# slp-rl/slamkit

Hardware: NVIDIA H100
Metric: speech-tokens/sec (SLAM seq=1024) (higher is better)
Workload: dtype bf16

## Files before the change

### slamkit_b200/csrc/attention.cu

```cuda
#include "kernels.h"

namespace {

constexpr int HD = 64;

SK_DEVINL uint32_t tile_addr(uint32_t base, int r, int chunk) { return base + r * 128 + ((chunk ^ (r & 7)) << 4); }
SK_DEVINL uint32_t smem_base_1k(const void* p) { return (smem_u32(p) + 1023u) & ~1023u; }

SK_DEVINL void cp_async16(uint32_t saddr, const void* g, bool pred) {
  const int sz = pred ? 16 : 0;
  asm volatile("cp.async.cg.shared.global [%0], [%1], 16, %2;" ::"r"(saddr), "l"(g), "r"(sz) : "memory");
}
SK_DEVINL void cp_async_commit() { asm volatile("cp.async.commit_group;" ::: "memory"); }
template <int N>
SK_DEVINL void cp_async_wait() {
  asm volatile("cp.async.wait_group %0;" ::"n"(N) : "memory");
}

SK_DEVINL void wgmma_m64n64_rs(float (&d)[32], const uint32_t (&a)[4], uint64_t db) {
  asm volatile(
      "{\n\t.reg .pred p;\n\tsetp.eq.u32 p, 1, 1;\n\t"
      "wgmma.mma_async.sync.aligned.m64n64k16.f32.bf16.bf16 {%0,%1,%2,%3,%4,%5,%6,%7,%8,%9,%10,%11,%12,%13,%14,%15,"
      "%16,%17,%18,%19,%20,%21,%22,%23,%24,%25,%26,%27,%28,%29,%30,%31}, {%32,%33,%34,%35}, %36, p, 1, 1, 1;\n\t}\n"
      : "+f"(d[0]), "+f"(d[1]), "+f"(d[2]), "+f"(d[3]), "+f"(d[4]), "+f"(d[5]), "+f"(d[6]), "+f"(d[7]), "+f"(d[8]),
// ... 18 lines not shown
  float(&d)[32] = reinterpret_cast<float(&)[32]>(acc);
  wgmma_fence();
#pragma unroll
  for (int ks = 0; ks < 4; ++ks)
    wgmma_m64n64<0, 0>(d, gmma_desc_sw128(sA + ks * 32, 16, 1024), gmma_desc_sw128(sB + ks * 32, 16, 1024));
  wgmma_commit();
  wgmma_wait<0>();
}

SK_DEVINL void wg_p_b(float (&acc)[8][4], const uint32_t (&p)[4][4], uint32_t sB) {
  float(&d)[32] = reinterpret_cast<float(&)[32]>(acc);
  wgmma_fence();
#pragma unroll
  for (int kk = 0; kk < 4; ++kk) wgmma_m64n64_rs(d, p[kk], gmma_desc_sw128(sB + kk * 2048, 8192, 1024));
  wgmma_commit();
  wgmma_wait<0>();
}

SK_DEVINL void acc_to_a(const float (&s)[8][4], uint32_t (&p)[4][4]) {
#pragma unroll
  for (int kk = 0; kk < 4; ++kk) {
    p[kk][0] = pack_bf16(s[2 * kk][0], s[2 * kk][1]);
    p[kk][1] = pack_bf16(s[2 * kk][2], s[2 * kk][3]);
    p[kk][2] = pack_bf16(s[2 * kk + 1][0], s[2 * kk + 1][1]);
    p[kk][3] = pack_bf16(s[2 * kk + 1][2], s[2 * kk + 1][3]);
  }
}

SK_DEVINL void zero_acc(float (&a)[8][4]) {
#pragma unroll
  for (int i = 0; i < 8; ++i)
#pragma unroll
    for (int j = 0; j < 4; ++j) a[i][j] = 0.f;
}

template <bool CAUSAL>
__global__ void __launch_bounds__(256, 2)
attn_fwd_kernel(const bf16* __restrict__ q, const bf16* __restrict__ k, const bf16* __restrict__ v, bf16* __restrict__ o,
                float* __restrict__ lse, int T, int ld, int ldo, int H, int group, float scale,
                const int* __restrict__ seg_start) {
  extern __shared__ __align__(128) uint8_t smem_attn[];
  const uint32_t sQ = smem_base_1k(smem_attn);
  const uint32_t sK = sQ + 128 * 128;
  const uint32_t sV = sK + 2 * 64 * 128;
  const int b = blockIdx.z, h = blockIdx.y;
  const int qt = gridDim.x - 1 - blockIdx.x;
  const int q0 = qt * 128;
  const int warp = threadIdx.x >> 5, lane = threadIdx.x & 31;
  const bf16* qp = q + (size_t)b * T * ld + h * HD;
  const bf16* kp = k + (size_t)b * T * ld + (h / group) * HD;
  const bf16* vp = v + (size_t)b * T * ld + (h / group) * HD;
  const float sl2 = scale * 1.4426950408889634f;

  int n_kv = (T + 63) / 64;
  if (CAUSAL) {
    const int last = min(T - 1, q0 + 127);
    n_kv = last / 64 + 1;
  }
  load_tile<128, 256>(sQ, qp, ld, q0, T);
  load_tile<64, 256>(sK, kp, ld, 0, T);
  load_tile<64, 256>(sV, vp, ld, 0, T);
  cp_async_commit();

  const uint32_t sQw = sQ + (uint32_t)(warp >> 2) * 8192u;
  float oacc[8][4];
  zero_acc(oacc);
// ... 249 lines not shown
    const long m = rh / H;
    const uint4 a = ldg128_stream(o + m * ldo + h * HD + part * 8);
    const uint4 g = ldg128_stream(d_o + m * ldo + h * HD + part * 8);
    const uint32_t au[4] = {a.x, a.y, a.z, a.w}, gu[4] = {g.x, g.y, g.z, g.w};
#pragma unroll
    for (int kq = 0; kq < 4; ++kq) {
      const float2 x = unpack_bf16(au[kq]), y = unpack_bf16(gu[kq]);
      acc += x.x * y.x + x.y * y.y;
    }
  }
  acc += __shfl_xor_sync(0xffffffffu, acc, 1);
  acc += __shfl_xor_sync(0xffffffffu, acc, 2);
  acc += __shfl_xor_sync(0xffffffffu, acc, 4);
  if (ok && (i & 7) == 0) {
    const int h = (int)(rh % H);
    const long m = rh / H;
    const long bb = m / T, t = m % T;
    delta[(bb * H + h) * T + t] = acc;
  }
}

template <bool CAUSAL>
__global__ void __launch_bounds__(128, 3)
attn_bwd_dkdv_kernel(const bf16* __restrict__ q, const bf16* __restrict__ k, const bf16* __restrict__ v,
                     const bf16* __restrict__ d_o, const float* __restrict__ lse, const float* __restrict__ delta,
                     bf16* __restrict__ dk, bf16* __restrict__ dv, int T, int ld, int ldo, int ldg, int H, int group,
                     float scale, const int* __restrict__ seg_start) {
  extern __shared__ __align__(128) uint8_t smem_attn[];
  const uint32_t sKV = smem_base_1k(smem_attn);
  const uint32_t sQ = sKV + 2 * 8192;
  const uint32_t sdO = sQ + 2 * 8192;
  float* sStat = reinterpret_cast<float*>(smem_attn + (sKV - smem_u32(smem_attn)) + 6 * 8192);
  int* sSeg = reinterpret_cast<int*>(sStat + 2 * 2 * 64);
  const int b = blockIdx.z, g = blockIdx.y;
  const int kt = blockIdx.x;
  const int k0 = kt * 64;
  const int warp = threadIdx.x >> 5, lane = threadIdx.x & 31;
  const float sl2 = scale * 1.4426950408889634f;
  const bf16* kp = k + (size_t)b * T * ld + g * HD;
  const bf16* vp = v + (size_t)b * T * ld + g * HD;

  load_tile<64, 128>(sKV, kp, ld, k0, T);
  load_tile<64, 128>(sKV + 8192, vp, ld, k0, T);
  cp_async_commit();

  const int n_qt = (T + 63) / 64;
  const int qt_begin = CAUSAL ? kt : 0;
  const int per_head = n_qt - qt_begin;
  const int n_iter = per_head * group;

  auto issue = [&](int it, int st) {
    const int h = g * group + it / per_head;
    const int qt = qt_begin + it % per_head;
    const bf16* qp = q + (size_t)b * T * ld + h * HD;
    const bf16* dop = d_o + (size_t)b * T * ldo + h * HD;
    load_tile<64, 128>(sQ + st * 8192, qp, ld, qt * 64, T);
    load_tile<64, 128>(sdO + st * 8192, dop, ldo, qt * 64, T);
    if (threadIdx.x < 64) {
      const int row = qt * 64 + threadIdx.x;
      const size_t off = ((size_t)b * H + h) * T + (row < T ? row : 0);
      sStat[(st * 2 + 0) * 64 + threadIdx.x] = row < T ? lse[off] : 0.f;
      sStat[(st * 2 + 1) * 64 + threadIdx.x] = row < T ? delta[off] : 0.f;
      sSeg[st * 64 + threadIdx.x] = (seg_start && row < T) ? seg_start[(size_t)b * T + row] : 0;
    }
    cp_async_commit();
  };
  if (n_iter > 0) issue(0, 0);

  float dkacc[8][4], dvacc[8][4];
  zero_acc(dkacc);
  zero_acc(dvacc);
  const int key_a = k0 + warp * 16 + (lane >> 2);

  for (int it = 0; it < n_iter; ++it) {
    const int st = it & 1;
    if (it + 1 < n_iter) {
      issue(it + 1, st ^ 1);
      cp_async_wait<1>();
    } else {
      cp_async_wait<0>();
    }
    __syncthreads();
    const int qt = qt_begin + it % per_head;
    const int q0 = qt * 64;
    const float* s_lse = sStat + (st * 2 + 0) * 64;
    const float* s_del = sStat + (st * 2 + 1) * 64;

    float st_acc[8][4];
    zero_acc(st_acc);
    wg_a_bT(st_acc, sKV, sQ + st * 8192);
    const int* s_seg = sSeg + st * 64;
    const bool need_mask = (CAUSAL && (q0 < k0 + 64)) || (q0 + 64 > T) || (k0 + 64 > T) || seg_start;
#pragma unroll
    for (int nt = 0; nt < 8; ++nt) {
#pragma unroll
      for (int e = 0; e < 4; ++e) {
        const int qi = nt * 8 + (lane & 3) * 2 + (e & 1);
        const int key = key_a + ((e >> 1) << 3);
        float pv = exp2f(st_acc[nt][e] * sl2 - s_lse[qi] * 1.4426950408889634f);
        if (need_mask) {
          const int qrow = q0 + qi;
          if (qrow >= T || key >= T || (CAUSAL && key > qrow) || key < s_seg[qi]) pv = 0.f;
        }
        st_acc[nt][e] = pv;
      }
    }
    uint32_t pa[4][4];
    acc_to_a(st_acc, pa);
    wg_p_b(dvacc, pa, sdO + st * 8192);

    float dp[8][4];
    zero_acc(dp);
    wg_a_bT(dp, sKV + 8192, sdO + st * 8192);
#pragma unroll
    for (int nt = 0; nt < 8; ++nt) {
#pragma unroll
      for (int e = 0; e < 4; ++e) {
        const int qi = nt * 8 + (lane & 3) * 2 + (e & 1);
        dp[nt][e] = st_acc[nt][e] * (dp[nt][e] - s_del[qi]) * scale;
      }
    }
    acc_to_a(dp, pa);
    wg_p_b(dkacc, pa, sQ + st * 8192);
    __syncthreads();
  }
#pragma unroll
  for (int r = 0; r < 2; ++r) {
    const int key = key_a + 8 * r;
    if (key < T) {
      bf16* dkp = dk + ((size_t)b * T + key) * ldg + g * HD;
      bf16* dvp = dv + ((size_t)b * T + key) * ldg + g * HD;
#pragma unroll
      for (int nt = 0; nt < 8; ++nt) {
        *reinterpret_cast<uint32_t*>(dkp + nt * 8 + (lane & 3) * 2) = pack_bf16(dkacc[nt][2 * r], dkacc[nt][2 * r + 1]);
        *reinterpret_cast<uint32_t*>(dvp + nt * 8 + (lane & 3) * 2) = pack_bf16(dvacc[nt][2 * r], dvacc[nt][2 * r + 1]);
      }
    }
  }
}

template <bool CAUSAL>
__global__ void __launch_bounds__(128)
attn_bwd_dq_kernel(const bf16* __restrict__ q, const bf16* __restrict__ k, const bf16* __restrict__ v,
                   const bf16* __restrict__ d_o, const float* __restrict__ lse, const float* __restrict__ delta,
                   bf16* __restrict__ dq, int T, int ld, int ldo, int ldg, int H, int group, float scale,
                   const int* __restrict__ seg_start) {
  extern __shared__ __align__(128) uint8_t smem_attn[];
  const uint32_t sQdO = smem_base_1k(smem_attn);
  const uint32_t sK = sQdO + 2 * 8192;
  const uint32_t sV = sK + 2 * 8192;
  const int b = blockIdx.z, h = blockIdx.y;
  const int qt = gridDim.x - 1 - blockIdx.x;
  const int q0 = qt * 64;
  const int warp = threadIdx.x >> 5, lane = threadIdx.x & 31;
  const float sl2 = scale * 1.4426950408889634f;
  const bf16* qp = q + (size_t)b * T * ld + h * HD;
  const bf16* dop = d_o + (size_t)b * T * ldo + h * HD;
  const bf16* kp = k + (size_t)b * T * ld + (h / group) * HD;
  const bf16* vp = v + (size_t)b * T * ld + (h / group) * HD;

  int n_kv = (T + 63) / 64;
  if (CAUSAL) n_kv = min(T - 1, q0 + 63) / 64 + 1;
  load_tile<64, 128>(sQdO, qp, ld, q0, T);
  load_tile<64, 128>(sQdO + 8192, dop, ldo, q0, T);
  load_tile<64, 128>(sK, kp, ld, 0, T);
  load_tile<64, 128>(sV, vp, ld, 0, T);
  cp_async_commit();

  const int row_a = q0 + warp * 16 + (lane >> 2);
  float lse_r[2], del_r[2];
  int seg_r[2];
#pragma unroll
  for (int r = 0; r < 2; ++r) {
    const int row = row_a + 8 * r;
    const size_t off = ((size_t)b * H + h) * T + (row < T ? row : 0);
    lse_r[r] = row < T ? lse[off] * 1.4426950408889634f : 0.f;
    del_r[r] = row < T ? delta[off] : 0.f;
    seg_r[r] = (seg_start && row < T) ? seg_start[(size_t)b * T + row] : 0;
  }
  float dqacc[8][4];
  zero_acc(dqacc);

  for (int j = 0; j < n_kv; ++j) {
    const int st = j & 1;
    if (j + 1 < n_kv) {
      load_tile<64, 128>(sK + (st ^ 1) * 8192, kp, ld, (j + 1) * 64, T);
      load_tile<64, 128>(sV + (st ^ 1) * 8192, vp, ld, (j + 1) * 64, T);
      cp_async_commit();
      cp_async_wait<1>();
    } else {
      cp_async_wait<0>();
    }
    __syncthreads();
    const int k0 = j * 64;
    float s[8][4];
    zero_acc(s);
    wg_a_bT(s, sQdO, sK + st * 8192);
    const bool need_mask = (CAUSAL && (k0 + 63 > q0 + warp * 16)) || (k0 + 64 > T) || (q0 + 64 > T) || seg_start;
#pragma unroll
    for (int nt = 0; nt < 8; ++nt) {
#pragma unroll
      for (int e = 0; e < 4; ++e) {
        float pv = exp2f(s[nt][e] * sl2 - lse_r[e >> 1]);
        if (need_mask) {
          const int key = k0 + nt * 8 + (lane & 3) * 2 + (e & 1);
          const int row = row_a + ((e >> 1) << 3);
          if (row >= T || key >= T || (CAUSAL && key > row) || key < seg_r[e >> 1]) pv = 0.f;
        }
        s[nt][e] = pv;
      }
    }
    float dp[8][4];
    zero_acc(dp);
    wg_a_bT(dp, sQdO + 8192, sV + st * 8192);
#pragma unroll
    for (int nt = 0; nt < 8; ++nt) {
#pragma unroll
      for (int e = 0; e < 4; ++e) dp[nt][e] = s[nt][e] * (dp[nt][e] - del_r[e >> 1]) * scale;
    }
    uint32_t pa[4][4];
    acc_to_a(dp, pa);
    wg_p_b(dqacc, pa, sK + st * 8192);
    __syncthreads();
  }
#pragma unroll
  for (int r = 0; r < 2; ++r) {
    const int row = row_a + 8 * r;
    if (row < T) {
      bf16* dqp = dq + ((size_t)b * T + row) * ldg + h * HD;
#pragma unroll
      for (int nt = 0; nt < 8; ++nt)
        *reinterpret_cast<uint32_t*>(dqp + nt * 8 + (lane & 3) * 2) = pack_bf16(dqacc[nt][2 * r], dqacc[nt][2 * r + 1]);
    }
  }
}

constexpr int FWD_SMEM = 128 * 128 + 4 * 8192 + 1024;
constexpr int DKDV_SMEM = 6 * 8192 + 2 * 2 * 64 * 4 + 2 * 64 * 4 + 1024;
constexpr int DQ_SMEM = 6 * 8192 + 1024;
constexpr int FWD_SPLIT_SMEM = 2 * 128 * 128 + 8 * 8192 + 1024;

template <typename K>
int set_smem(K kernel, int bytes) {
  SK_CUDA_CHECK(cudaFuncSetAttribute(kernel, cudaFuncAttributeMaxDynamicSharedMemorySize, bytes));
  return 0;
}

// ... 10 lines not shown
    if (set_smem(attn_fwd_kernel<true>, FWD_SMEM)) return -2;
    if (set_smem(attn_fwd_kernel<false>, FWD_SMEM)) return -2;
    init = true;
  }
  dim3 grid((T + 127) / 128, H, B);
  sk_prof_begin(1, s);
  if (causal) attn_fwd_kernel<true><<<grid, 256, FWD_SMEM, s>>>(q, k, v, o, lse, T, ld, ldo, H, H / KVH, scale, seg_start);
  else attn_fwd_kernel<false><<<grid, 256, FWD_SMEM, s>>>(q, k, v, o, lse, T, ld, ldo, H, H / KVH, scale, nullptr);
  sk_prof_end(s);
  SK_LAUNCH_CHECK();
  return 0;
}

int sk_attn_bwd_launch(const bf16* q, const bf16* k, const bf16* v, const bf16* o, const bf16* d_o, const float* lse,
                       float* delta, bf16* dq, bf16* dk, bf16* dv, int B, int T, int H, int KVH, int ld, int ldo,
                       int ldg, int causal, float scale, cudaStream_t s, const int* seg_start) {
  SK_REQUIRE(seg_start == nullptr || causal, "attention: document segments need the causal kernels");
  SK_REQUIRE(B > 0 && T > 0 && H > 0 && KVH > 0, "attention: bad shape B=%d T=%d H=%d KVH=%d", B, T, H, KVH);
  SK_REQUIRE(H % KVH == 0, "attention: H must be a multiple of KVH");
  SK_REQUIRE(ld % 8 == 0 && ldo % 8 == 0 && ldg % 2 == 0, "attention: ld and ldo must be multiples of 8 and ldg even");
  static bool init = false;
  if (!init) {
    if (set_smem(attn_bwd_dkdv_kernel<true>, DKDV_SMEM)) return -2;
    if (set_smem(attn_bwd_dkdv_kernel<false>, DKDV_SMEM)) return -2;
    if (set_smem(attn_bwd_dq_kernel<true>, DQ_SMEM)) return -2;
    if (set_smem(attn_bwd_dq_kernel<false>, DQ_SMEM)) return -2;
    init = true;
  }
  const long total = (long)B * T * H * 8;
  sk_prof_begin(1, s);
  SK_CUDA_CHECK(sk_launch_pdl(attn_delta_kernel, dim3((int)((total + 255) / 256)), dim3(256), (size_t)(0), s, o, d_o, delta, B, T, H, ldo));
  SK_LAUNCH_CHECK();
  const int group = H / KVH;
  dim3 g1((T + 63) / 64, KVH, B), g2((T + 63) / 64, H, B);
  if (causal) {
    attn_bwd_dkdv_kernel<true><<<g1, 128, DKDV_SMEM, s>>>(q, k, v, d_o, lse, delta, dk, dv, T, ld, ldo, ldg, H, group, scale,
                                                          seg_start);
    SK_LAUNCH_CHECK();
    attn_bwd_dq_kernel<true><<<g2, 128, DQ_SMEM, s>>>(q, k, v, d_o, lse, delta, dq, T, ld, ldo, ldg, H, group, scale, seg_start);
  } else {
    attn_bwd_dkdv_kernel<false><<<g1, 128, DKDV_SMEM, s>>>(q, k, v, d_o, lse, delta, dk, dv, T, ld, ldo, ldg, H, group, scale,
                                                           nullptr);
    SK_LAUNCH_CHECK();
    attn_bwd_dq_kernel<false><<<g2, 128, DQ_SMEM, s>>>(q, k, v, d_o, lse, delta, dq, T, ld, ldo, ldg, H, group, scale, nullptr);
  }
  sk_prof_end(s);
  SK_LAUNCH_CHECK();
  return 0;
}

int sk_attn_fwd_split_launch(const bf16* q_hi, const bf16* q_lo, const bf16* k_hi, const bf16* k_lo, const bf16* v_hi,
                             const bf16* v_lo, bf16* o_hi, bf16* o_lo, int B, int T, int H, int ld, int ldo, float scale,
                             cudaStream_t s) {
  SK_REQUIRE(B > 0 && T > 0 && H > 0, "attention: bad shape B=%d T=%d H=%d", B, T, H);
  SK_REQUIRE(ld % 8 == 0 && ldo % 8 == 0, "attention: leading dims must be multiples of 8");
  static bool init = false;
  if (!init) {
    if (set_smem(attn_fwd_split_kernel, FWD_SPLIT_SMEM)) return -2;
    init = true;
  }
  dim3 grid((T + 127) / 128, H, B);
  sk_prof_begin(1, s);
  attn_fwd_split_kernel<<<grid, 256, FWD_SPLIT_SMEM, s>>>(q_hi, q_lo, k_hi, k_lo, v_hi, v_lo, o_hi, o_lo, T, ld, ldo, scale);
  sk_prof_end(s);
  SK_LAUNCH_CHECK();
  return 0;
}
// ... 36 lines not shown
```

### slamkit_b200/csrc/gemm_tcgen05.cu

```cuda
#include "common.cuh"
#include <cudaTypedefs.h>
#include <stdio.h>
#include <mutex>
#include <type_traits>
#include <string.h>
#include <stdlib.h>
#include "kernels.h"
#include "../../include/slamkit_b200.h"

namespace {

constexpr int BM = 128;
constexpr int BK = 64;
constexpr int MMA_K = 16;
constexpr int GEMM_THREADS = 288;


struct GemmParams {
  int M, N, K;
  int batch;
  int a_mode;
  int passes;
  void* C;
  void* C_lo;
  int ldc;
  const void* bias;
  int bias_f32;
  const bf16* residual;
  const bf16* residual_lo;
  int ldr;
  int tiles_m, tiles_n;
  int out_f32;
  int round_before_res;
  int act;
  int col_gin, col_gout;
  int splits;
  float* splitk_ws;
  int tma_store;
  int pdl;
  int sk_units;
  int sk_groups;
  int sk_G;
  int sk_colunits;
  int sk_carry;
  int units, n_groups;
  float* sk_ws;
  uint32_t* sk_flags;
  int epi;
  const bf16* aux;
  int ld_aux;
  const bf16* rope_cos;
  const bf16* rope_sin;
  const int* rope_pos;
  int rope_T, rope_cols, rope_maxpos, rope_rot;
};

template <int BN, int EW = 4>
struct GemmCfg {
  static constexpr int A_BYTES = BM * BK * 2;
  static constexpr int B_ATOMS = (BN + 63) / 64;
  static constexpr int B_BYTES = B_ATOMS * 64 * BK * 2;
  static constexpr int STAGE_BYTES = A_BYTES + B_BYTES;
  static constexpr int STAGES = (BN > 128) ? 4 : (BN > 64 ? 6 : 8);
  static constexpr int STAGING_BYTES = 4 * 2 * 4096;
  static constexpr int BAR_BYTES = 256;
  static constexpr int SMEM_BYTES = STAGES * STAGE_BYTES + STAGING_BYTES + BAR_BYTES + 1024;
  static_assert(BN % 64 == 0 || (BN == 224 && EW == 4), "a 32-column tail chunk only on the 224-wide tile");
  static_assert(STAGES * STAGE_BYTES >= BM * BN * 4, "the parked fp32 accumulator must fit in the stage ring");
  static_assert(SMEM_BYTES <= 227 * 1024, "sm_90 allows 227 KB of shared memory per block");
};

// ... 17 lines not shown
template <int BN>
SK_DEVINL void acc_ld_32x32(uint32_t base, uint32_t ta, uint32_t (&r)[32]) {
  const int row = (int)(ta >> 16) + (int)(threadIdx.x & 31);
  const int c0 = (int)(ta & 0xffffu) >> 2;
#pragma unroll
  for (int i = 0; i < 8; ++i)
    asm volatile("ld.shared.v4.b32 {%0, %1, %2, %3}, [%4];"
                 : "=r"(r[4 * i]), "=r"(r[4 * i + 1]), "=r"(r[4 * i + 2]), "=r"(r[4 * i + 3])
                 : "r"(acc_chunk_addr<BN>(base, row, c0 + i)) : "memory");
}

SK_DEVINL uint32_t staging_addr(uint32_t sbuf, int lane, int j, bool tail) {
  return tail ? sbuf + (uint32_t)lane * 64u + (uint32_t)((j ^ ((lane >> 1) & 3)) << 4)
              : sbuf + (uint32_t)lane * 128u + (uint32_t)((j ^ (lane & 7)) << 4);
}

SK_DEVINL float gelu_erf(float y) {
  const float a = fabsf(y);
  float t;
  asm("rcp.approx.ftz.f32 %0, %1;" : "=f"(t) : "f"(fmaf(0.3275911f * 0.70710678118654752440f, a, 1.0f)));
  float s = fmaf(0.5f * 1.061405429f, t, 0.5f * -1.453152027f);
  s = fmaf(s, t, 0.5f * 1.421413741f);
  s = fmaf(s, t, 0.5f * -0.284496736f);
  s = fmaf(s, t, 0.5f * 0.254829592f);
  const float e = ex2_approx((y * y) * -0.72134752044448170368f);
  return fmaf(-a, (s * t) * e, fmaxf(y, 0.0f));
}

SK_DEVINL float gelu_exact(float x) { return x * 0.5f * (1.0f + erff(x * 0.70710678118654752440f)); }
SK_DEVINL float gelu_exact_grad(float x) {
  const float cdf = 0.5f * (1.0f + erff(x * 0.70710678118654752440f));
  const float pdf = expf(-0.5f * x * x) * 0.39894228040143267794f;
  return cdf + x * pdf;
}

template <bool SK>
struct WorkIter {
  int num_kb, splits, kb_per_split, total_items, tiles_n;
  int G, colunits, carry, units, n_groups, sk_groups, grp, mem;
  long sk_total, sk_cur, sk_end;
  int next_unit, next_item;
  int tile, split, kb_begin, kb_end, role;
  long unit_end_it;
  SK_DEVINL WorkIter(const GemmParams& p, int num_kb_, int kb_per_split_, int total_items_) {
    num_kb = num_kb_;
    splits = p.splits;
    kb_per_split = kb_per_split_;
    total_items = total_items_;
    tiles_n = p.tiles_n;
    G = p.sk_G;
    colunits = p.sk_colunits;
    carry = p.sk_carry;
    units = p.units;
    n_groups = p.n_groups;
    sk_groups = p.sk_groups;
    tile = split = kb_begin = kb_end = role = 0;
    unit_end_it = 0;
    sk_total = sk_cur = sk_end = 0;
    next_item = (int)blockIdx.x;
    next_unit = 0;
    grp = mem = 0;
    if (SK && p.sk_units > 0) {
      grp = (int)blockIdx.x / G;
      mem = (int)blockIdx.x - grp * G;
      next_item = total_items;
      next_unit = grp < n_groups ? p.sk_units + grp : units;
// ... 172 lines not shown

  const int warp = threadIdx.x >> 5;
  const int lane = threadIdx.x & 31;
  const int tiles_per_batch = p.tiles_m * p.tiles_n;
  const int total_items = tiles_per_batch * p.batch * p.splits;
  const int num_kb_total = (p.K + BK - 1) / BK;
  const int kb_per_split = (num_kb_total + p.splits - 1) / p.splits;
  constexpr uint32_t STAGE_TX = Cfg::A_BYTES + (B_MN ? Cfg::B_ATOMS * 64 * BK * 2 : BN * BK * 2);

  if (threadIdx.x == 0) {
    tma_prefetch_desc(&tmA);
    tma_prefetch_desc(&tmB);
    for (int s = 0; s < Cfg::STAGES; ++s) {
      mbar_init(full_bar(s), 1);
      mbar_init(empty_bar(s), 8);
    }
    mbar_init(acc_free, 1);
    fence_mbar_init();
  }
  __syncthreads();
  griddep_wait();

  if (warp == 8) {
    if (lane == 0) {
      const bool split = p.passes == 3;
      const int n_stage = split ? Cfg::STAGES / 2 : Cfg::STAGES;
      const uint32_t stage_bytes = split ? 2u * Cfg::STAGE_BYTES : (uint32_t)Cfg::STAGE_BYTES;
      int stage = 0;
      uint32_t phase = 0;
      uint32_t acc_phase = 0;
      bool first = true;
      WorkIter<SK> w(p, num_kb_total, kb_per_split, total_items);
      while (w.next()) {
        if (!first) {
          mbar_wait_nocall(acc_free, acc_phase);
          acc_phase ^= 1u;
        }
        first = false;
        const int bidx = w.tile / tiles_per_batch;
        const int r = w.tile - bidx * tiles_per_batch;
        const int m0 = (r / p.tiles_n) * BM;
        const int n_blk = r % p.tiles_n;
        const int n0 = n_blk * BN;
        for (int kb = w.kb_begin; kb < w.kb_end; ++kb) {
          mbar_wait_nocall(empty_bar(stage), phase ^ 1u);
          const uint32_t fb = full_bar(stage);
          mbar_arrive_expect_tx(fb, split ? 2u * STAGE_TX : STAGE_TX);
          for (int part = 0; part < (split ? 2 : 1); ++part) {
            const CUtensorMap* mapA = part ? &tmA_lo : &tmA;
            const CUtensorMap* mapB = part ? &tmB_lo : &tmB;
            const uint32_t sA = smem_base + stage * stage_bytes + part * Cfg::STAGE_BYTES;
            const uint32_t sB = sA + Cfg::A_BYTES;
            if (!A_MN) {
              if (p.a_mode & 2) {
                if (p.a_mode & 1) tma_load_3d(sA, mapA, fb, n_blk * 64, m0 + kb, bidx);
                else tma_load_3d(sA, mapA, fb, kb * BK, m0, bidx);
              } else {
                tma_load_2d(sA, mapA, fb, kb * BK, m0);
              }
            } else {
#pragma unroll
              for (int j = 0; j < BM / 64; ++j) tma_load_2d(sA + j * (BK * 128), mapA, fb, m0 + 64 * j, kb * BK);
            }
            if (!B_MN) {
              tma_load_2d(sB, mapB, fb, kb * BK, n0);
            } else {
#pragma unroll
              for (int j = 0; j < Cfg::B_ATOMS; ++j) tma_load_2d(sB + j * (BK * 128), mapB, fb, n0 + 64 * j, kb * BK);
            }
          }
          if (++stage == n_stage) { stage = 0; phase ^= 1u; }
        }
      }
    }
  } else {
    const int wg = warp >> 2;
    const int q = warp & 3;
    const int chalf = warp >> 2;
    const bool epi_warp = warp < EW;
    auto acc_ld = [&](uint32_t ta, uint32_t (&r)[32]) { acc_ld_32x32<BN>(smem_base, ta, r); };
    const bool split = p.passes == 3;
    const int n_stage = split ? Cfg::STAGES / 2 : Cfg::STAGES;
    const uint32_t stage_bytes = split ? 2u * Cfg::STAGE_BYTES : (uint32_t)Cfg::STAGE_BYTES;
    int stage = 0;
    uint32_t phase = 0;
    uint32_t store_cnt = 0;
    auto release_acc = [&] {
      fence_proxy_async();
      named_bar_sync(1, 256);
      if (threadIdx.x == 0) mbar_arrive(acc_free);
    };
    WorkIter<SK> w(p, num_kb_total, kb_per_split, total_items);
    while (w.next()) {
      {
        float acc[BN / 2];
#pragma unroll
        for (int i = 0; i < BN / 2; ++i) acc[i] = 0.f;
        if (SK && w.role == 3) {
          const int src = (int)blockIdx.x - w.G;
          if (threadIdx.x == 0) {
            for (int qq = 0; qq < 4; ++qq) {
              const uint32_t* f = p.sk_flags + src * 4 + qq;
              const uint64_t t0 = globaltimer_ns();
              while (ld_acquire_u32(f) == 0u) {
                __nanosleep(64);
                if (globaltimer_ns() - t0 > 8000000000ull) __trap();
              }
            }
            for (int qq = 0; qq < 4; ++qq) p.sk_flags[src * 4 + qq] = 0u;
          }
          named_bar_sync(1, 256);
          const float* slot = p.sk_ws + (size_t)src * SK_SLOT_FLOATS;
          const int r0 = 64 * wg + 16 * (warp & 3) + (lane >> 2);
#pragma unroll
          for (int j = 0; j < BN / 8; ++j) {
            const int col = 8 * j + 2 * (lane & 3);
#pragma unroll
            for (int h = 0; h < 2; ++h) {
              const float2 v = __ldcg(reinterpret_cast<const float2*>(slot + sk_slot_off(col >> 5, (col & 31) >> 2, r0 + 8 * h) +
                                                                      (col & 3)));
              acc[4 * j + 2 * h] = v.x;
              acc[4 * j + 2 * h + 1] = v.y;
            }
          }
        }
        const int k_iters = max(0, w.kb_end - w.kb_begin);
        int prev = -1;
        for (int kb = 0; kb < k_iters; ++kb) {
          mbar_wait_nocall(full_bar(stage), phase);
          wgmma_fence();
          const uint32_t s_hi = smem_base + stage * stage_bytes;
          for (int g = 0; g < (split ? 3 : 1); ++g) {
            const uint32_t sA = s_hi + (g == 2 ? Cfg::STAGE_BYTES : 0) + (uint32_t)wg * 8192u;
            const uint32_t sB = s_hi + Cfg::A_BYTES + (g == 1 ? Cfg::STAGE_BYTES : 0);
#pragma unroll
            for (int k = 0; k < BK / MMA_K; ++k) {
              const uint64_t adesc = A_MN ? gmma_desc_sw128(sA + k * (MMA_K * 128), BK * 128, 1024)
                                          : gmma_desc_sw128(sA + k * (MMA_K * 2), 16, 1024);
              const uint64_t bdesc = B_MN ? gmma_desc_sw128(sB + k * (MMA_K * 128), BK * 128, 1024)
                                          : gmma_desc_sw128(sB + k * (MMA_K * 2), 16, 1024);
              wgmma_bf16<BN, A_MN ? 1 : 0, B_MN ? 1 : 0>(acc, adesc, bdesc);
            }
          }
          wgmma_commit();
          wgmma_wait<1>();
          if (prev >= 0 && lane == 0) mbar_arrive(empty_bar(prev));
          prev = stage;
          if (++stage == n_stage) { stage = 0; phase ^= 1u; }
        }
        wgmma_wait<0>();
        if (prev >= 0 && lane == 0) mbar_arrive(empty_bar(prev));
        named_bar_sync(1, 256);
        acc_park<BN>(smem_base, acc, wg, warp & 3, lane);
        named_bar_sync(1, 256);
      }
      if (!epi_warp) {
        release_acc();
        continue;
      }
      const int split_idx = w.split;
      const int bidx = w.tile / tiles_per_batch;
      const int rr = w.tile - bidx * tiles_per_batch;
      const int m0 = (rr / p.tiles_n) * BM;
      const int n0 = (rr % p.tiles_n) * BN;
      if (!SK && p.tma_store && p.epi == 2) {
        const int lpiece = lane & 7, lrsub = lane >> 3;
        const uint32_t sX = staging_base + (uint32_t)warp * (EW == 4 ? 8192u : 4096u);
        constexpr int NCH = BN / 64 / CS;
        const int c_lo = chalf * NCH;
        auto piece_off = [&](int bidx, int m0, int n0, int c2, size_t ld) -> size_t {
          const int acol = n0 + c2 * 64;
          const int gcol = (acol >> 7) * 256 + (acol & 127) + lpiece * 8;
          return (((size_t)bidx * p.M + m0 + q * 32 + lrsub) * ld + gcol) * sizeof(bf16);
        };
        const size_t row4_in = (size_t)4 * p.ld_aux * sizeof(bf16), row4_out = (size_t)4 * p.ldc * sizeof(bf16);
        uint4 gv[8], uv[8];
        auto gu_load_k = [&](int k, const uint8_t* base, int m0, int n0, int c2) {
          const int rin = m0 + q * 32 + 4 * k + lrsub;
          if (rin < p.M && n0 + c2 * 64 < p.N) {
            gv[k] = ldg128(base + k * row4_in);
            uv[k] = ldg128(base + k * row4_in + 256);
          } else {
            gv[k] = make_uint4(0u, 0u, 0u, 0u);
            uv[k] = make_uint4(0u, 0u, 0u, 0u);
          }
        };
        {
          const uint8_t* base = reinterpret_cast<const uint8_t*>(p.aux) + piece_off(bidx, m0, n0, c_lo, (size_t)p.ld_aux);
// ... 462 lines not shown
                if (p.out_f32) {
                  float* dst = reinterpret_cast<float*>(p.C) + row * p.ldc + ocol;
                  *reinterpret_cast<float4*>(dst) = make_float4(v[0], v[1], v[2], v[3]);
                  *reinterpret_cast<float4*>(dst + 4) = make_float4(v[4], v[5], v[6], v[7]);
                } else {
                  uint4 o;
                  o.x = pack_bf16(v[0], v[1]);
                  o.y = pack_bf16(v[2], v[3]);
                  o.z = pack_bf16(v[4], v[5]);
                  o.w = pack_bf16(v[6], v[7]);
                  stg128(reinterpret_cast<bf16*>(p.C) + row * p.ldc + ocol, o);
                  if (p.C_lo) {
                    const float2 h0 = unpack_bf16(o.x), h1 = unpack_bf16(o.y), h2 = unpack_bf16(o.z), h3 = unpack_bf16(o.w);
                    uint4 l;
                    l.x = pack_bf16(v[0] - h0.x, v[1] - h0.y);
                    l.y = pack_bf16(v[2] - h1.x, v[3] - h1.y);
                    l.z = pack_bf16(v[4] - h2.x, v[5] - h2.y);
                    l.w = pack_bf16(v[6] - h3.x, v[7] - h3.y);
                    stg128(reinterpret_cast<bf16*>(p.C_lo) + row * p.ldc + ocol, l);
                  }
                }
              }
            }
          }
        }
        if (SK && w.role == 2) {
          __syncwarp();
          if (lane == 0)
            for (int i = 0; i < n_contrib; ++i) p.sk_flags[(first_contrib + i * w.G) * 4 + q] = 0u;
        }
      }
      release_acc();
    }
    if (epi_warp && p.tma_store && lane == 0) tma_store_wait<0>();
  }
}

__global__ void splitk_reduce_kernel(const float* __restrict__ ws, bf16* __restrict__ C, int M, int N, int ldc, int splits,
                                     int accumulate, int round_before_res) {
  griddep_launch();
  griddep_wait();
  const long total = (long)M * N / 8;
  for (long i = blockIdx.x * (long)blockDim.x + threadIdx.x; i < total; i += (long)gridDim.x * blockDim.x) {
    const long e = i * 8;
    const int m = (int)(e / N), n = (int)(e % N);
    float acc[8] = {0, 0, 0, 0, 0, 0, 0, 0};
    for (int s = 0; s < splits; ++s) {
      const float* src = ws + ((size_t)s * M + m) * N + n;
      const float4 a = *reinterpret_cast<const float4*>(src), b = *reinterpret_cast<const float4*>(src + 4);
      acc[0] += a.x; acc[1] += a.y; acc[2] += a.z; acc[3] += a.w;
      acc[4] += b.x; acc[5] += b.y; acc[6] += b.z; acc[7] += b.w;
    }
    bf16* dst = C + (size_t)m * ldc + n;
    if (accumulate) {
      const uint4 o = *reinterpret_cast<const uint4*>(dst);
      const uint32_t ow[4] = {o.x, o.y, o.z, o.w};
#pragma unroll
      for (int k = 0; k < 4; ++k) {
        const float2 f = unpack_bf16(ow[k]);
        acc[2 * k] = (round_before_res ? bf16_round(acc[2 * k]) : acc[2 * k]) + f.x;
        acc[2 * k + 1] = (round_before_res ? bf16_round(acc[2 * k + 1]) : acc[2 * k + 1]) + f.y;
      }
    }
    stg128(dst, make_uint4(pack_bf16(acc[0], acc[1]), pack_bf16(acc[2], acc[3]), pack_bf16(acc[4], acc[5]),
                           pack_bf16(acc[6], acc[7])));
  }
}
// ... 234 lines not shown
    }
  }
  p.sk_G = 1;
  if (sk_ok && BN == 256 && p.splits == 1 && num_kb >= sk_min_kb && (p.tiles_n <= 8 || p.tiles_m <= 8)) {
    const int colunits = p.tiles_n <= 8 ? 0 : 1;
    const int G = colunits ? p.tiles_m : p.tiles_n;
    const int units = colunits ? p.tiles_n : p.tiles_m;
    const int n_groups = nsm / G;
    const int rem = units % n_groups;
    const long slots = ((long)(units + n_groups - 1) / n_groups) * n_groups;
    const bool multiwave = units > n_groups;
    if (n_groups >= 1 && rem != 0 && (slots - units) * 100 >= slots * sk_min_idle &&
        (!colunits || multiwave || sk_env >= 2)) {
      if (colunits && multiwave) {
        p.sk_units = rem + n_groups;
        p.sk_groups = n_groups;
        p.sk_carry = 1;
      } else {
        p.sk_units = rem;
        p.sk_groups = n_groups < rem * sk_ranges ? n_groups : rem * sk_ranges;
      }
      p.sk_G = G;
      p.sk_colunits = colunits;
      p.units = units;
      p.n_groups = n_groups;
      p.sk_ws = reinterpret_cast<float*>(g.splitk_ws);
      p.sk_flags = reinterpret_cast<uint32_t*>(reinterpret_cast<uint8_t*>(g.splitk_ws) + ws_data_bytes);
    }
  }
  const long work = tiles * p.splits;
  grid = p.sk_units > 0 ? p.n_groups * p.sk_G : (int)(work < nsm ? work : nsm);
  static const int ew_env = [] { const char* e = getenv("SK_GEMM_EW"); return e ? atoi(e) : 0; }();
  ew = (p.sk_units == 0 && BN == 256 && p.tma_store && (ew_env == 8 || (ew_env == 0 && (g.epi == 2 || g.epi == 3 || g.epi == 4 || g.epi == 5)))) ? 8 : 4;
  return 0;
}

}

int sk_gemm_plan_ex(const SkGemmEx& g, SkGemmPlan* out) {
  GemmParams p;
  int BN = 0, ew = 0, grid = 0;
  const int rc = plan_gemm(g, p, BN, ew, grid);
  if (rc) return rc;
  out->bn = BN;
  out->epi_warps = ew;
  out->splits = p.splits;
  out->sk_units = p.sk_units;
  out->sk_groups = p.sk_groups;
  out->sk_G = p.sk_G;
  out->sk_colunits = p.sk_colunits;
  out->tma_store = p.tma_store;
  out->grid = grid;
  return 0;
}

int sk_gemm_ex_launch(const SkGemmEx& g, cudaStream_t stream) {
  GemmParams p;
  int BN = 0, ew = 0, grid = 0;
  const int rc0 = plan_gemm(g, p, BN, ew, grid);
  if (rc0) return rc0;
  const bool use3d = g.a_rows > 0;
  CUtensorMap tm[6];
  const void* As[2] = {g.A, g.passes == 3 ? g.A_lo : g.A};
  const void* Bs[2] = {g.B, g.passes == 3 ? g.B_lo : g.B};
  for (int i = 0; i < 2; ++i) {
    int rc;
    CUtensorMap* ta = &tm[i == 0 ? 0 : 2];
    CUtensorMap* tb = &tm[i == 0 ? 1 : 3];
    if (use3d) {
      rc = sk_make_tmap_3d(ta, As[i], (uint64_t)g.a_inner, (uint64_t)g.a_rows, (uint64_t)g.batch, (uint64_t)g.a_row_stride,
                           (uint64_t)g.a_batch_stride, BM);
    } else if (!g.a_mn) {
      rc = sk_make_tmap_2d(ta, As[i], 2, (uint64_t)g.K, (uint64_t)g.M, (uint64_t)g.lda, BK, BM);
    } else {
      rc = sk_make_tmap_2d(ta, As[i], 2, (uint64_t)g.M, (uint64_t)g.K, (uint64_t)g.lda, 64, BK);
    }
    if (rc) return rc;
    if (!g.b_mn) rc = sk_make_tmap_2d(tb, Bs[i], 2, (uint64_t)g.K, (uint64_t)g.N, (uint64_t)g.ldb, BK, (uint32_t)BN);
    else         rc = sk_make_tmap_2d(tb, Bs[i], 2, (uint64_t)g.N, (uint64_t)g.K, (uint64_t)g.ldb, 64, BK);
    if (rc) return rc;
  }
  tm[4] = tm[0];
  if (p.tma_store) {
    const int rc2 = sk_make_tmap_2d(&tm[4], g.C, 2, (uint64_t)(g.epi == 2 ? 2 * g.N : g.N), (uint64_t)g.M, (uint64_t)g.ldc, 64, 32);
    if (rc2) return rc2;
  }
  tm[5] = tm[4];
  if (g.epi == 1) {
    const int rc3 = sk_make_tmap_2d(&tm[5], g.aux_out, 2, (uint64_t)g.N / 2, (uint64_t)g.M, (uint64_t)g.ld_aux_out, 64, 32);
    if (rc3) return rc3;
  } else if (g.epi == 4) {
    const int rc3 = sk_make_tmap_2d(&tm[5], g.aux_out, 2, (uint64_t)g.N, (uint64_t)g.M, (uint64_t)g.ld_aux_out, 64, 32);
    if (rc3) return rc3;
  } else if (p.tma_store && BN % 64 != 0) {
    const int rc3 = sk_make_tmap_2d(&tm[5], g.C, 2, (uint64_t)g.N, (uint64_t)g.M, (uint64_t)g.ldc, 32, 32);
    if (rc3) return rc3;
  }
  int rc;
  if (p.sk_units > 0) {
    rc = dispatch_major<256, true>(g.a_mn, g.b_mn, tm, p, grid, stream);
  } else if (ew == 8) {
    rc = dispatch_major<256, false, 8>(g.a_mn, g.b_mn, tm, p, grid, stream);
  } else {
    switch (BN) {
      case 256: rc = dispatch_major<256, false>(g.a_mn, g.b_mn, tm, p, grid, stream); break;
      case 224: rc = dispatch_major<224, false>(g.a_mn, g.b_mn, tm, p, grid, stream); break;
      case 192: rc = dispatch_major<192, false>(g.a_mn, g.b_mn, tm, p, grid, stream); break;
      case 128: rc = dispatch_major<128, false>(g.a_mn, g.b_mn, tm, p, grid, stream); break;
      default:  rc = dispatch_major<64, false>(g.a_mn, g.b_mn, tm, p, grid, stream); break;
    }
  }
  if (rc) return rc;
  if (p.splits > 1) {
    SK_REQUIRE(g.residual == nullptr || g.residual == g.C, "gemm: split-K supports only in-place accumulation");
    const long n8 = (long)g.M * g.N / 8;
    int blocks = (int)((n8 + 255) / 256);
    if (blocks > sk_num_sms() * 8) blocks = sk_num_sms() * 8;
    sk_prof_begin(0, stream);
    SK_CUDA_CHECK(sk_launch_pdl(splitk_reduce_kernel, dim3(blocks), dim3(256), (size_t)(0), stream, p.splitk_ws, reinterpret_cast<bf16*>(g.C), g.M, g.N, g.ldc, p.splits,
                                                     g.residual != nullptr, g.round_before_res));
    sk_prof_end(stream);
    SK_LAUNCH_CHECK();
  }
  return 0;
}

SkGemmEx sk_gemm_desc(int M, int N, int K, const void* A, int lda, int a_mn, const void* B, int ldb, int b_mn, void* C,
                      int ldc, int out_f32, const void* bias, const void* residual, int ldr, int round_before_res, int act,
// ... 85 lines not shown
```

Measured before the change: 153,700.

## Overlap independent wgmma groups in attention backward and reorder dK/dV grid

In both backward kernels the S=QK^T and dP=dO·V^T matmuls are now issued back to back as separate async wgmma groups. The softmax/mask math on the first runs while the second is still in flight, and in dK/dV the dV update is also issued asynchronously before dS is computed. The dK/dV grid is flattened to one dimension with key tile as the slowest index, which changes the scheduling order across heads and batches. The dQ kernel gets a min-blocks launch bound of 4, which raises register pressure because two accumulators are now live at once.

```diff
diff --git a/slamkit_b200/csrc/attention.cu b/slamkit_b200/csrc/attention.cu
--- a/slamkit_b200/csrc/attention.cu
+++ b/slamkit_b200/csrc/attention.cu
@@ -74,6 +74,21 @@
   for (int i = 0; i < 8; ++i)
 #pragma unroll
     for (int j = 0; j < 4; ++j) a[i][j] = 0.f;
+}
+
+SK_DEVINL void wg_a_bT_async(float (&acc)[8][4], uint32_t sA, uint32_t sB) {
+  float(&d)[32] = reinterpret_cast<float(&)[32]>(acc);
+#pragma unroll
+  for (int ks = 0; ks < 4; ++ks)
+    wgmma_m64n64<0, 0>(d, gmma_desc_sw128(sA + ks * 32, 16, 1024), gmma_desc_sw128(sB + ks * 32, 16, 1024));
+  wgmma_commit();
+}
+
+SK_DEVINL void acc_fence(float (&a)[8][4]) {
+#pragma unroll
+  for (int i = 0; i < 8; ++i)
+#pragma unroll
+    for (int j = 0; j < 4; ++j) asm volatile("" : "+f"(a[i][j])::"memory");
 }
 
 template <bool CAUSAL>
@@ -389,8 +404,11 @@
   const uint32_t sdO = sQ + 2 * 8192;
   float* sStat = reinterpret_cast<float*>(smem_attn + (sKV - smem_u32(smem_attn)) + 6 * 8192);
   int* sSeg = reinterpret_cast<int*>(sStat + 2 * 2 * 64);
-  const int b = blockIdx.z, g = blockIdx.y;
-  const int kt = blockIdx.x;
+  const int n_qt = (T + 63) / 64;
+  const int kvh = H / group;
+  const int per_kt = gridDim.x / n_qt;
+  const int kt = blockIdx.x / per_kt;
+  const int g = blockIdx.x % per_kt % kvh, b = blockIdx.x % per_kt / kvh;
   const int k0 = kt * 64;
   const int warp = threadIdx.x >> 5, lane = threadIdx.x & 31;
   const float sl2 = scale * 1.4426950408889634f;
@@ -401,7 +419,6 @@
   load_tile<64, 128>(sKV + 8192, vp, ld, k0, T);
   cp_async_commit();
 
-  const int n_qt = (T + 63) / 64;
   const int qt_begin = CAUSAL ? kt : 0;
   const int per_head = n_qt - qt_begin;
   const int n_iter = per_head * group;
@@ -444,8 +461,16 @@
     const float* s_del = sStat + (st * 2 + 1) * 64;
 
     float st_acc[8][4];
+    float dp[8][4];
     zero_acc(st_acc);
-    wg_a_bT(st_acc, sKV, sQ + st * 8192);
+    zero_acc(dp);
+    acc_fence(st_acc);
+    acc_fence(dp);
+    wgmma_fence();
+    wg_a_bT_async(st_acc, sKV, sQ + st * 8192);
+    wg_a_bT_async(dp, sKV + 8192, sdO + st * 8192);
+    wgmma_wait<1>();
+    acc_fence(st_acc);
     const int* s_seg = sSeg + st * 64;
     const bool need_mask = (CAUSAL && (q0 < k0 + 64)) || (q0 + 64 > T) || (k0 + 64 > T) || seg_start;
 #pragma unroll
@@ -464,11 +489,16 @@
     }
     uint32_t pa[4][4];
     acc_to_a(st_acc, pa);
-    wg_p_b(dvacc, pa, sdO + st * 8192);
-
-    float dp[8][4];
-    zero_acc(dp);
-    wg_a_bT(dp, sKV + 8192, sdO + st * 8192);
+    wgmma_fence();
+    {
+      float(&d)[32] = reinterpret_cast<float(&)[32]>(dvacc);
+#pragma unroll
+      for (int kk = 0; kk < 4; ++kk)
+        wgmma_m64n64_rs(d, pa[kk], gmma_desc_sw128(sdO + st * 8192 + kk * 2048, 8192, 1024));
+      wgmma_commit();
+    }
+    wgmma_wait<1>();
+    acc_fence(dp);
 #pragma unroll
     for (int nt = 0; nt < 8; ++nt) {
 #pragma unroll
@@ -477,6 +507,7 @@
         dp[nt][e] = st_acc[nt][e] * (dp[nt][e] - s_del[qi]) * scale;
       }
     }
+    wgmma_wait<0>();
     acc_to_a(dp, pa);
     wg_p_b(dkacc, pa, sQ + st * 8192);
     __syncthreads();
@@ -497,7 +528,7 @@
 }
 
 template <bool CAUSAL>
-__global__ void __launch_bounds__(128)
+__global__ void __launch_bounds__(128, 4)
 attn_bwd_dq_kernel(const bf16* __restrict__ q, const bf16* __restrict__ k, const bf16* __restrict__ v,
                    const bf16* __restrict__ d_o, const float* __restrict__ lse, const float* __restrict__ delta,
                    bf16* __restrict__ dq, int T, int ld, int ldo, int ldg, int H, int group, float scale,
@@ -550,9 +581,16 @@
     }
     __syncthreads();
     const int k0 = j * 64;
-    float s[8][4];
+    float s[8][4], dp[8][4];
     zero_acc(s);
-    wg_a_bT(s, sQdO, sK + st * 8192);
+    zero_acc(dp);
+    acc_fence(s);
+    acc_fence(dp);
+    wgmma_fence();
+    wg_a_bT_async(s, sQdO, sK + st * 8192);
+    wg_a_bT_async(dp, sQdO + 8192, sV + st * 8192);
+    wgmma_wait<1>();
+    acc_fence(s);
     const bool need_mask = (CAUSAL && (k0 + 63 > q0 + warp * 16)) || (k0 + 64 > T) || (q0 + 64 > T) || seg_start;
 #pragma unroll
     for (int nt = 0; nt < 8; ++nt) {
@@ -567,9 +605,8 @@
         s[nt][e] = pv;
       }
     }
-    float dp[8][4];
-    zero_acc(dp);
-    wg_a_bT(dp, sQdO + 8192, sV + st * 8192);
+    wgmma_wait<0>();
+    acc_fence(dp);
 #pragma unroll
     for (int nt = 0; nt < 8; ++nt) {
 #pragma unroll
@@ -646,7 +683,9 @@
   SK_CUDA_CHECK(sk_launch_pdl(attn_delta_kernel, dim3((int)((total + 255) / 256)), dim3(256), (size_t)(0), s, o, d_o, delta, B, T, H, ldo));
   SK_LAUNCH_CHECK();
   const int group = H / KVH;
-  dim3 g1((T + 63) / 64, KVH, B), g2((T + 63) / 64, H, B);
+  const long n_dkdv = (long)((T + 63) / 64) * KVH * B;
+  SK_REQUIRE(n_dkdv < (1l << 31), "attention: %ld dK/dV tiles exceed one grid dimension", n_dkdv);
+  dim3 g1((unsigned)n_dkdv), g2((T + 63) / 64, H, B);
   if (causal) {
     attn_bwd_dkdv_kernel<true><<<g1, 128, DKDV_SMEM, s>>>(q, k, v, d_o, lse, delta, dk, dv, T, ld, ldo, ldg, H, group, scale,
                                                           seg_start);
```

Result: no change. 155,200 (median of 6 runs) (+0.9%).

## Store GEMM epilogue directly from registers via stmatrix and TMA, skipping accumulator park

Applied to the files above, without the earlier changes.

For plain and SwiGLU-gated epilogues with no bias, activation or residual, the math warpgroups now pack accumulators to bf16 themselves. They write them into per-warp staging buffers with stmatrix and issue 16-row TMA stores. This removes the shared-memory accumulator park, the handoff to separate epilogue warps, and the producer's wait on acc_free. In exchange, consumer warps now spend time on the epilogue, so the next tile's mainloop no longer overlaps with the previous tile's stores. The staging-buffer layout and swizzle must also match the new 16-row TMA box.

```diff
diff --git a/slamkit_b200/csrc/gemm_tcgen05.cu b/slamkit_b200/csrc/gemm_tcgen05.cu
--- a/slamkit_b200/csrc/gemm_tcgen05.cu
+++ b/slamkit_b200/csrc/gemm_tcgen05.cu
@@ -37,6 +37,7 @@
   int splits;
   float* splitk_ws;
   int tma_store;
+  int reg_epi;
   int pdl;
   int sk_units;
   int sk_groups;
@@ -120,6 +121,11 @@
   const float cdf = 0.5f * (1.0f + erff(x * 0.70710678118654752440f));
   const float pdf = expf(-0.5f * x * x) * 0.39894228040143267794f;
   return cdf + x * pdf;
+}
+
+SK_DEVINL void stmatrix_x4(uint32_t addr, uint32_t a, uint32_t b, uint32_t c, uint32_t d) {
+  asm volatile("stmatrix.sync.aligned.m8n8.x4.shared.b16 [%0], {%1, %2, %3, %4};" ::"r"(addr), "r"(a), "r"(b), "r"(c),
+               "r"(d) : "memory");
 }
 
 template <bool SK>
@@ -358,7 +364,7 @@
       bool first = true;
       WorkIter<SK> w(p, num_kb_total, kb_per_split, total_items);
       while (w.next()) {
-        if (!first) {
+        if (!first && !p.reg_epi) {
           mbar_wait_nocall(acc_free, acc_phase);
           acc_phase ^= 1u;
         }
@@ -419,10 +425,104 @@
     WorkIter<SK> w(p, num_kb_total, kb_per_split, total_items);
     while (w.next()) {
       {
-        float acc[BN / 2];
-#pragma unroll
-        for (int i = 0; i < BN / 2; ++i) acc[i] = 0.f;
+        auto reg_epilogue = [&](const float (&acc)[BN / 2]) {
+          const int rr = w.tile;
+          const int m0 = (rr / p.tiles_n) * BM, n0 = (rr % p.tiles_n) * BN;
+          const int row0 = m0 + 16 * warp;
+          const uint32_t stg = staging_base + (uint32_t)warp * 4096u;
+          auto emit = [&](const uint32_t (&pk)[16], const CUtensorMap* map, int col, bool tail) {
+            const uint32_t sbuf = stg + (store_cnt & 1u) * 2048u;
+            if (lane == 0) tma_store_wait_read<1>();
+            __syncwarp();
+            const int srow = (lane & 7) + (lane & 8);
+#pragma unroll
+            for (int jj = 0; jj < (tail ? 4 : 8); jj += 2) {
+              const int ch = jj + (lane >> 4);
+              const uint32_t addr = tail ? sbuf + (uint32_t)srow * 64u + (uint32_t)((ch ^ ((srow >> 1) & 3)) << 4)
+                                         : sbuf + (uint32_t)srow * 128u + (uint32_t)((ch ^ (srow & 7)) << 4);
+              stmatrix_x4(addr, pk[2 * jj], pk[2 * jj + 1], pk[2 * jj + 2], pk[2 * jj + 3]);
+            }
+            fence_proxy_async();
+            __syncwarp();
+            if (lane == 0) {
+              tma_store_2d(map, sbuf, col, row0);
+              tma_store_commit();
+            }
+            ++store_cnt;
+          };
+          auto pair_bf16 = [&](int j, int h) { return pack_bf16(acc[4 * j + 2 * h], acc[4 * j + 2 * h + 1]); };
+          if (p.epi == 1) {
+            if constexpr (BN == 256) {
+#pragma unroll
+              for (int i = 0; i < 2; ++i) {
+                uint32_t pk[16];
+#pragma unroll
+                for (int t = 0; t < 16; ++t) pk[t] = pair_bf16(8 * i + (t >> 1), t & 1);
+                emit(pk, &tmC, n0 + 64 * i, false);
+#pragma unroll
+                for (int t = 0; t < 16; ++t) pk[t] = pair_bf16(16 + 8 * i + (t >> 1), t & 1);
+                emit(pk, &tmC, n0 + 128 + 64 * i, false);
+#pragma unroll
+                for (int t = 0; t < 16; ++t) {
+                  const float2 gf = unpack_bf16(pair_bf16(8 * i + (t >> 1), t & 1));
+                  const float2 uf = unpack_bf16(pair_bf16(16 + 8 * i + (t >> 1), t & 1));
+                  const float2 sb = unpack_bf16(pack_bf16(silu_f(gf.x), silu_f(gf.y)));
+                  pk[t] = pack_bf16(sb.x * uf.x, sb.y * uf.y);
+                }
+                emit(pk, &tmAux, (n0 >> 1) + 64 * i, false);
+              }
+            }
+          } else {
+#pragma unroll
+            for (int c2 = 0; c2 < (BN + 63) / 64; ++c2) {
+              const bool tail = BN % 64 != 0 && c2 == BN / 64;
+              if (n0 + 64 * c2 >= p.N) continue;
+              uint32_t pk[16];
+#pragma unroll
+              for (int t = 0; t < (tail ? 8 : 16); ++t) pk[t] = pair_bf16(8 * c2 + (t >> 1), t & 1);
+              emit(pk, tail ? &tmAux : &tmC, n0 + 64 * c2, tail);
+            }
+          }
+        };
+        auto mainloop_park = [&](float (&acc)[BN / 2]) {
+          const int k_iters = max(0, w.kb_end - w.kb_begin);
+          int prev = -1;
+          for (int kb = 0; kb < k_iters; ++kb) {
+            mbar_wait_nocall(full_bar(stage), phase);
+            wgmma_fence();
+            const uint32_t s_hi = smem_base + stage * stage_bytes;
+            for (int g = 0; g < (split ? 3 : 1); ++g) {
+              const uint32_t sA = s_hi + (g == 2 ? Cfg::STAGE_BYTES : 0) + (uint32_t)wg * 8192u;
+              const uint32_t sB = s_hi + Cfg::A_BYTES + (g == 1 ? Cfg::STAGE_BYTES : 0);
+#pragma unroll
+              for (int k = 0; k < BK / MMA_K; ++k) {
+                const uint64_t adesc = A_MN ? gmma_desc_sw128(sA + k * (MMA_K * 128), BK * 128, 1024)
+                                            : gmma_desc_sw128(sA + k * (MMA_K * 2), 16, 1024);
+                const uint64_t bdesc = B_MN ? gmma_desc_sw128(sB + k * (MMA_K * 128), BK * 128, 1024)
+                                            : gmma_desc_sw128(sB + k * (MMA_K * 2), 16, 1024);
+                wgmma_bf16<BN, A_MN ? 1 : 0, B_MN ? 1 : 0>(acc, adesc, bdesc);
+              }
+            }
+            wgmma_commit();
+            wgmma_wait<1>();
+            if (prev >= 0 && lane == 0) mbar_arrive(empty_bar(prev));
+            prev = stage;
+            if (++stage == n_stage) { stage = 0; phase ^= 1u; }
+          }
+          wgmma_wait<0>();
+          if (prev >= 0 && lane == 0) mbar_arrive(empty_bar(prev));
+          if constexpr (!SK && EW == 4) {
+            if (p.reg_epi) {
+              reg_epilogue(acc);
+              return;
+            }
+          }
+          named_bar_sync(1, 256);
+          acc_park<BN>(smem_base, acc, wg, warp & 3, lane);
+          named_bar_sync(1, 256);
+        };
         if (SK && w.role == 3) {
+          float acc[BN / 2];
           const int src = (int)blockIdx.x - w.G;
           if (threadIdx.x == 0) {
             for (int qq = 0; qq < 4; ++qq) {
@@ -449,37 +549,15 @@
               acc[4 * j + 2 * h + 1] = v.y;
             }
           }
+          mainloop_park(acc);
+        } else {
+          float acc[BN / 2];
+#pragma unroll
+          for (int i = 0; i < BN / 2; ++i) acc[i] = 0.f;
+          mainloop_park(acc);
         }
-        const int k_iters = max(0, w.kb_end - w.kb_begin);
-        int prev = -1;
-        for (int kb = 0; kb < k_iters; ++kb) {
-          mbar_wait_nocall(full_bar(stage), phase);
-          wgmma_fence();
-          const uint32_t s_hi = smem_base + stage * stage_bytes;
-          for (int g = 0; g < (split ? 3 : 1); ++g) {
-            const uint32_t sA = s_hi + (g == 2 ? Cfg::STAGE_BYTES : 0) + (uint32_t)wg * 8192u;
-            const uint32_t sB = s_hi + Cfg::A_BYTES + (g == 1 ? Cfg::STAGE_BYTES : 0);
-#pragma unroll
-            for (int k = 0; k < BK / MMA_K; ++k) {
-              const uint64_t adesc = A_MN ? gmma_desc_sw128(sA + k * (MMA_K * 128), BK * 128, 1024)
-                                          : gmma_desc_sw128(sA + k * (MMA_K * 2), 16, 1024);
-              const uint64_t bdesc = B_MN ? gmma_desc_sw128(sB + k * (MMA_K * 128), BK * 128, 1024)
-                                          : gmma_desc_sw128(sB + k * (MMA_K * 2), 16, 1024);
-              wgmma_bf16<BN, A_MN ? 1 : 0, B_MN ? 1 : 0>(acc, adesc, bdesc);
-            }
-          }
-          wgmma_commit();
-          wgmma_wait<1>();
-          if (prev >= 0 && lane == 0) mbar_arrive(empty_bar(prev));
-          prev = stage;
-          if (++stage == n_stage) { stage = 0; phase ^= 1u; }
-        }
-        wgmma_wait<0>();
-        if (prev >= 0 && lane == 0) mbar_arrive(empty_bar(prev));
-        named_bar_sync(1, 256);
-        acc_park<BN>(smem_base, acc, wg, warp & 3, lane);
-        named_bar_sync(1, 256);
       }
+      if (!SK && p.reg_epi) continue;
       if (!epi_warp) {
         release_acc();
         continue;
@@ -1008,7 +1086,7 @@
       }
       release_acc();
     }
-    if (epi_warp && p.tma_store && lane == 0) tma_store_wait<0>();
+    if ((epi_warp || p.reg_epi) && p.tma_store && lane == 0) tma_store_wait<0>();
   }
 }
 
@@ -1309,6 +1387,7 @@
   grid = p.sk_units > 0 ? p.n_groups * p.sk_G : (int)(work < nsm ? work : nsm);
   static const int ew_env = [] { const char* e = getenv("SK_GEMM_EW"); return e ? atoi(e) : 0; }();
   ew = (p.sk_units == 0 && BN == 256 && p.tma_store && (ew_env == 8 || (ew_env == 0 && (g.epi == 2 || g.epi == 3 || g.epi == 4 || g.epi == 5)))) ? 8 : 4;
+  p.reg_epi = (p.tma_store && p.sk_units == 0 && ew == 4 && !g.bias && !g.act && !g.residual && (g.epi == 0 || g.epi == 1)) ? 1 : 0;
   return 0;
 }
 
@@ -1358,19 +1437,20 @@
     if (rc) return rc;
   }
   tm[4] = tm[0];
+  const uint32_t box_rows = p.reg_epi ? 16 : 32;
   if (p.tma_store) {
-    const int rc2 = sk_make_tmap_2d(&tm[4], g.C, 2, (uint64_t)(g.epi == 2 ? 2 * g.N : g.N), (uint64_t)g.M, (uint64_t)g.ldc, 64, 32);
+    const int rc2 = sk_make_tmap_2d(&tm[4], g.C, 2, (uint64_t)(g.epi == 2 ? 2 * g.N : g.N), (uint64_t)g.M, (uint64_t)g.ldc, 64, box_rows);
     if (rc2) return rc2;
   }
   tm[5] = tm[4];
   if (g.epi == 1) {
-    const int rc3 = sk_make_tmap_2d(&tm[5], g.aux_out, 2, (uint64_t)g.N / 2, (uint64_t)g.M, (uint64_t)g.ld_aux_out, 64, 32);
+    const int rc3 = sk_make_tmap_2d(&tm[5], g.aux_out, 2, (uint64_t)g.N / 2, (uint64_t)g.M, (uint64_t)g.ld_aux_out, 64, box_rows);
     if (rc3) return rc3;
   } else if (g.epi == 4) {
     const int rc3 = sk_make_tmap_2d(&tm[5], g.aux_out, 2, (uint64_t)g.N, (uint64_t)g.M, (uint64_t)g.ld_aux_out, 64, 32);
     if (rc3) return rc3;
   } else if (p.tma_store && BN % 64 != 0) {
-    const int rc3 = sk_make_tmap_2d(&tm[5], g.C, 2, (uint64_t)g.N, (uint64_t)g.M, (uint64_t)g.ldc, 32, 32);
+    const int rc3 = sk_make_tmap_2d(&tm[5], g.C, 2, (uint64_t)g.N, (uint64_t)g.M, (uint64_t)g.ldc, 32, box_rows);
     if (rc3) return rc3;
   }
   int rc;
```

New measurement: 153,300 before, 161,600 after, median of 6. 1.05x the previous value.
